# iqbal-lab-org/gramtools

Measured on AMD Instinct MI355X. Metric: 150bp reads quasimapped/sec (whole node); bit-exact coverage, higher is better.
Workload: dtype u32

## Files before the change

gramtools_amd/csrc/gmx_engine_cover_kernels.h:

```cpp
#pragma once
struct CoverAcc {
  uint32_t *acc;
  uint32_t *log;
  uint32_t *log_cursor;
  uint32_t log_cap;
  uint32_t *scratch_big;
  uint32_t n_lanes_big;
  int rng_mode;
  uint32_t log_sites;
  uint32_t *heap;
  uint64_t heap_words;
  const uint32_t *status;
  uint32_t n_tasks;
  unsigned long long *stats;
};

#define GMX_LOG_PAD 0xFFFFFFFFu
#ifdef GMX_LOOP_STATS
__device__ unsigned long long gmx_cover_stats[6 * 16];
__device__ unsigned long long gmx_coop_stats[6 * 8];
extern "C" int gmx_debug_coop_stats(unsigned long long *out, int reset) {
  if (hipMemcpyFromSymbol(out, HIP_SYMBOL(gmx_coop_stats), sizeof(gmx_coop_stats)) != hipSuccess) return -1;
  if (reset) {
    unsigned long long z[6 * 8] = {0};
// ... 800 lines not shown
    c[GMX_CNT_LOG_RETRY_HUGE * GMX_CNT_STRIDE] = 0;
  }
}
template <bool NESTED>
__global__ void __launch_bounds__(GMX_BLOCK) gmx_cover_single_replay_kernel(GmxIndexView ix, BatchView b, SearchOut o, CoverAcc acc,
                                                                            const uint32_t *recs_in) {
  const uint32_t n = o.counters[GMX_CNT_REPLAY_RECS * GMX_CNT_STRIDE];
  for (uint32_t i = blockIdx.x * GMX_BLOCK + threadIdx.x; i < n; i += gridDim.x * GMX_BLOCK)
    gmx_cover_single_rec<NESTED>(ix, o, acc, recs_in[i], o.cover_overflow_list, 4u);
}

__global__ void gmx_stats_limbs_kernel(unsigned long long *stats, uint32_t *limbs, int recombine) {
  const uint32_t t = threadIdx.x;
  if (!recombine) {
    if (t < 20) limbs[t] = (uint32_t)((stats[t >> 2] >> (16 * (t & 3))) & 0xFFFFull);
    else if (t < 32) limbs[t] = 0;
  } else if (t < 5) {
    unsigned long long v = 0;
    for (int l = 3; l >= 0; --l) v = (v << 16) + limbs[4 * t + l];
    stats[t] = v;
  }
}

#define GMX_PACK_READS 128
#define GMX_PACK_IN_BYTES (24 * 1024)
#define GMX_PACK_OUT_PAIRS (GMX_PACK_IN_BYTES / 32 + GMX_PACK_READS + 8)
typedef uint32_t __attribute__((aligned(1))) gmx_u32_unaligned;
__device__ __forceinline__ void pack4(uint32_t x, uint32_t &lo, uint32_t &hi, uint32_t &bad) {
  uint32_t y = x - 0x01010101u;
  bad |= ((y & ~x & 0x80808080u) | (y & 0xFCFCFCFCu));
  lo = (((y & 0x01010101u) * 0x01020408u) >> 24) & 0xFu;
  hi = ((((y >> 1) & 0x01010101u) * 0x01020408u) >> 24) & 0xFu;
}
__device__ __forceinline__ uint2 pack_tail(const uint8_t *p, uint32_t rem, uint32_t &bad) {
  uint2 out = make_uint2(0, 0);
  for (uint32_t j = 0; j < rem; ++j) {
    uint32_t x = p[j];
    if (x < 1 || x > 4) bad = 1;
    out.x |= ((x - 1u) & 1u) << j;
    out.y |= (((x - 1u) >> 1) & 1u) << j;
  }
  return out;
}
#define GMX_PACK_THREADS (2 * GMX_PACK_READS)
__global__ void __launch_bounds__(GMX_PACK_THREADS) gmx_pack_kernel(BatchView b, uint8_t *skip, uint2 *packed, uint32_t *counters,
                                                                    uint32_t *zero, uint32_t zero_words) {
// ... 86 lines not shown
```

gramtools_amd/csrc/gmx_engine_host.h:

```cpp
#pragma once
#define HIP_TRY(expr)                                                                      \
  do {                                                                                     \
    hipError_t _e = (expr);                                                                \
    if (_e != hipSuccess) {                                                                \
      gmx_set_error(std::string(#expr) + ": " + hipGetErrorString(_e));                    \
      return GMX_EHIP;                                                                     \
    }                                                                                      \
  } while (0)

enum : int { GMX_TK_SEED = 0, GMX_TK_FILTER0, GMX_TK_FILTER1, GMX_TK_SINGLE, GMX_TK_EXTEND2, GMX_TK_UNPACK, GMX_TK_N };
static_assert(GMX_TK_N <= GMX_TIMED_KERNELS, "gmx_timing::kernel_ms holds GMX_TIMED_KERNELS entries");

struct gmx_engine {
  gmx_engine_opts opts;
  GmxIndexView dview;
  std::vector<void *> allocs;
  uint64_t index_bytes = 0;
  uint32_t *d_fused = nullptr, *d_limbs = nullptr;
  size_t n_fused = 0, n_acc = 0;
  std::vector<uint32_t> phys_allele, phys_pb, phys_grouped;
  std::vector<uint32_t> hit_fix;
  unsigned long long *d_stats = nullptr;
  uint32_t *d_error = nullptr;
  uint32_t *d_log = nullptr, *d_log_cursor = nullptr;
  uint32_t log_cap = 0;
  uint32_t n_allele = 0, n_pb = 0, n_grouped = 0;
  uint64_t cap_reads = 0;
  uint8_t *d_skip = nullptr;
  uint2 *d_packed = nullptr;
  uint64_t cap_packed = 0;
  uint32_t *d_status = nullptr, *d_n_final = nullptr, *d_mapped = nullptr, *d_overflow = nullptr, *d_counters = nullptr;
  uint32_t *d_general_rest = nullptr;
  uint32_t *d_single_rest = nullptr;
  bool cover_jump = false;
  uint32_t *d_task_lists = nullptr;
  GmxSeed *d_alive_seed = nullptr;
  uint32_t *d_alive = nullptr, *d_dead = nullptr, *d_dead2 = nullptr;
  uint64_t *d_seed_cursor = nullptr;
  bool seed_cursor = false;
  GmxFinalState *d_finals = nullptr;
  GmxPathNode *d_arena = nullptr;
  GmxCoverRec *d_cover_recs = nullptr;
  BigOut big{};
  uint32_t *d_scratch_big = nullptr, *d_cover_overflow = nullptr;
  uint32_t cover_big_lanes = 0;
// ... 3 lines not shown
  uint32_t inst_cap = 0;
  GmxPathNode *d_inst_arena = nullptr;
  GmxFinalState *d_inst_states = nullptr;
  uint32_t *d_inst_first = nullptr, *d_inst_width = nullptr;
  uint32_t *d_inst_serial = nullptr, *d_general_serial = nullptr, *d_big_serial = nullptr, *d_overflow3 = nullptr;
  bool coop = true;
  uint32_t *d_heap = nullptr;
  uint64_t heap_words = 0;
  bool log_sites = false;
  std::map<std::vector<uint32_t>, uint64_t> log_counts;
  uint32_t *h_log_state = nullptr;
  hipEvent_t ev_log_state = nullptr;
  bool log_state_pending = false;
  uint32_t *d_log_retry[2] = {nullptr, nullptr}, *d_log_retry_recs[2] = {nullptr, nullptr}, *d_log_retry_huge[2] = {nullptr, nullptr};
  int log_retry_side = 0;
  BatchView last_b{};
  SearchOut last_o{};
  CoverAcc last_acc{};
  size_t last_big_lds = 0;
  uint64_t log_replays = 0, log_replayed_entries = 0;
  uint64_t log_known = 0;
  uint64_t log_reads_since = 0;
  bool reset_pending = false;
  hipStream_t reset_stream = nullptr;
  hipStream_t side2_stream = nullptr;
  hipEvent_t ev_fork2 = nullptr, ev_side1 = nullptr, ev_filter = nullptr;
  hipStream_t side_stream = nullptr;
  hipEvent_t ev_fork = nullptr, ev_join = nullptr;
  hipEvent_t ev_wait = nullptr;
  struct GmxDeviceIndex *shared_index = nullptr;
  uint32_t filter_lds_words = 0;
  const uint32_t *d_kmer_planar = nullptr;
  const uint32_t *d_absent = nullptr;
  uint32_t n_absent = 0;
  bool use_absent = false;
  uint32_t n_cus = 256;
  uint32_t probe_iters = GMX_PROBE_ITERS;
  uint32_t extend_cap = 0;
  uint32_t extend_budget = 8;
  bool seeds_in_place = false;
  gmx_engine *twin = nullptr;
  gmx_engine *owner = nullptr;
  bool is_twin = false, twin_off = false;
  bool record_outcomes = false;
  uint32_t *d_outcomes = nullptr;
  uint64_t outcome_cap = 0, outcome_count = 0;
// ... 16 lines not shown
  uint64_t *d_offsets = nullptr;
  uint32_t *d_seeds = nullptr;
  uint64_t cap_bases = 0, cap_stage_reads = 0;
  struct StageSlot {
    uint8_t *d_reads = nullptr;
    uint64_t *d_offsets = nullptr, *h_offsets = nullptr;
    uint32_t *d_seeds = nullptr, *h_seeds = nullptr;
    uint64_t cap_bases = 0, cap_reads = 0;
    hipEvent_t copied = nullptr, done = nullptr;
    bool busy = false;
  } stage[2];
  hipStream_t copy_stream = nullptr;
  hipStream_t copy_stream2 = nullptr;
  uint32_t copy_toggle = 0;
  hipStream_t last_stream = nullptr;
  struct PackSlot {
    uint2 *d_planes = nullptr;
    uint64_t *d_offsets = nullptr;
    uint32_t *d_seeds = nullptr;
    uint8_t *d_skip = nullptr;
    uint64_t cap_pairs = 0, cap_reads = 0;
    hipEvent_t copied = nullptr, done = nullptr;
    bool busy = false;
  } pslot[3];
  uint32_t pslot_next = 0;
  void release(void *q) {
    if (!q) return;
    for (size_t i = 0; i < allocs.size(); ++i)
      if (allocs[i] == q) {
        allocs[i] = allocs.back();
        allocs.pop_back();
        (void)hipFree(q);
        return;
      }
  }
  bool timing = false;
  struct EvTriple { hipEvent_t s, a, b, c; uint64_t reads; hipEvent_t k[GMX_TIMED_KERNELS][2]; uint32_t timed; };
  std::vector<EvTriple> pending;
  double search_ms = 0, cover_ms = 0;
  uint64_t search_launches = 0, cover_launches = 0, timed_reads = 0;
  double kernel_ms[GMX_TIMED_KERNELS] = {0};
  uint64_t kernel_launches[GMX_TIMED_KERNELS] = {0};

  template <class T>
  int alloc(T **p, size_t count, bool zero) {
    void *q = nullptr;
    size_t bytes = std::max<size_t>(count, 1) * sizeof(T);
    allocs.reserve(allocs.size() + 1);
// ... 56 lines not shown
  }
  return GMX_OK;
}

static int note_zeroed(gmx_engine *e, hipStream_t stream) {
  if (!e->twin) return GMX_OK;
  if (!e->ev_zeroed) HIP_TRY(hipEventCreateWithFlags(&e->ev_zeroed, hipEventDisableTiming));
  HIP_TRY(hipEventRecord(e->ev_zeroed, stream));
  ++e->zero_epoch;
  return GMX_OK;
}
static int twin_join(gmx_engine *e, hipStream_t stream) {
  gmx_engine *tw = e->twin;
  if (!tw || !e->twin_in_flight) return GMX_OK;
  if (!e->ev_twin_done) HIP_TRY(hipEventCreateWithFlags(&e->ev_twin_done, hipEventDisableTiming));
  HIP_TRY(hipEventRecord(e->ev_twin_done, tw->main_stream));
  HIP_TRY(hipStreamWaitEvent(stream, e->ev_twin_done, 0));
  return GMX_OK;
}
static int flush_reset(gmx_engine *e) {
  if (!e->reset_pending) return GMX_OK;
  e->reset_pending = false;
  HIP_TRY(hipMemsetAsync(e->d_fused, 0, (e->n_fused + 32) * 4, e->reset_stream));
  return note_zeroed(e, e->reset_stream);
}

static int log_settle(gmx_engine *e);
static int gmx_log_drain(gmx_engine *e, uint64_t keep_below) {
  int frc = flush_reset(e);
  if (frc) return frc;
  HIP_TRY(hipDeviceSynchronize());
  uint32_t used = 0;
  HIP_TRY(hipMemcpy(&used, e->d_log_cursor, 4, hipMemcpyDeviceToHost));
  used = std::min(used, e->log_cap);
  e->log_reads_since = 0;
  e->log_known = used;
  if (used <= keep_below) return GMX_OK;
  std::vector<uint32_t> w(used);
  HIP_TRY(hipMemcpy(w.data(), e->d_log, (size_t)used * 4, hipMemcpyDeviceToHost));
  std::vector<uint32_t> key;
  for (size_t i = 0; i < w.size();) {
    if (w[i] == GMX_LOG_PAD) {
      ++i;
      continue;
    }
    if (i + 2 > w.size() || i + 2 + (size_t)w[i + 1] > w.size()) {
      gmx_set_error("grouped-allele-count log: malformed record at word " + std::to_string(i) + " of " + std::to_string(w.size()));
      return GMX_EREF;
// ... 432 lines not shown
    return GMX_EHIP;
  }
  *out = e;
  return GMX_OK;
}

void gmx_engine_destroy(gmx_engine *e) try {
  if (!e) return;
  (void)hipSetDevice(e->opts.device);
  (void)hipDeviceSynchronize();
  if (e->twin) gmx_engine_destroy(e->twin);
  e->twin = nullptr;
  if (e->main_stream) (void)hipStreamDestroy(e->main_stream);
  if (e->ev_zeroed) (void)hipEventDestroy(e->ev_zeroed);
  if (e->ev_twin_done) (void)hipEventDestroy(e->ev_twin_done);
  if (e->side_stream) (void)hipStreamDestroy(e->side_stream);
  if (e->side2_stream) (void)hipStreamDestroy(e->side2_stream);
  if (e->ev_fork2) (void)hipEventDestroy(e->ev_fork2);
  if (e->ev_side1) (void)hipEventDestroy(e->ev_side1);
  if (e->ev_filter) (void)hipEventDestroy(e->ev_filter);
  if (e->ev_fork) (void)hipEventDestroy(e->ev_fork);
  if (e->ev_join) (void)hipEventDestroy(e->ev_join);
  if (e->ev_wait) (void)hipEventDestroy(e->ev_wait);
  if (e->copy_stream) (void)hipStreamDestroy(e->copy_stream);
  if (e->copy_stream2) (void)hipStreamDestroy(e->copy_stream2);
  if (e->h_log_state) (void)hipHostFree(e->h_log_state);
  if (e->ev_log_state) (void)hipEventDestroy(e->ev_log_state);
  for (auto &sl : e->pslot) {
    if (sl.copied) (void)hipEventDestroy(sl.copied);
    if (sl.done) (void)hipEventDestroy(sl.done);
  }
  for (auto &sl : e->stage) {
    if (sl.copied) (void)hipEventDestroy(sl.copied);
    if (sl.done) (void)hipEventDestroy(sl.done);
    if (sl.h_offsets) (void)hipHostFree(sl.h_offsets);
    if (sl.h_seeds) (void)hipHostFree(sl.h_seeds);
  }
  for (void *p : e->allocs) (void)hipFree(p);
  if (e->d_outcomes) (void)hipFree(e->d_outcomes);
  gmx_dev_index_release(e->shared_index);
  delete e;
} GMX_GUARD_VOID("gmx_engine_destroy")

int gmx_engine_reset(gmx_engine *e) try {
  HIP_TRY(hipSetDevice(e->opts.device));
  e->reset_pending = false;
  HIP_TRY(hipDeviceSynchronize());
  HIP_TRY(hipMemset(e->d_fused, 0, (e->n_fused + 32) * 4));
  HIP_TRY(hipMemset(e->d_error, 0, 8));
  HIP_TRY(hipMemset(e->d_counters, 0, GMX_N_COUNTERS * GMX_CNT_STRIDE * 4));
  if (e->twin) {
    HIP_TRY(hipMemset(e->twin->d_error, 0, 8));
    HIP_TRY(hipMemset(e->twin->d_counters, 0, GMX_N_COUNTERS * GMX_CNT_STRIDE * 4));
    e->twin_in_flight = false;
  }
  if (e->outcome_count) HIP_TRY(hipMemset(e->d_outcomes, 0, (e->outcome_count + 3) & ~3ull));
  e->outcome_count = 0;
  ++e->outcome_epoch;
  e->log_counts.clear();
  e->log_known = e->log_reads_since = 0;
  e->log_state_pending = false;
  return GMX_OK;
} GMX_GUARD_INT("gmx_engine_reset")

int gmx_engine_reset_async(gmx_engine *e, void *hip_stream) try {
  HIP_TRY(hipSetDevice(e->opts.device));
  hipStream_t st = (hipStream_t)hip_stream;
  int frc = flush_reset(e);
  if (frc) return frc;
  if ((frc = twin_join(e, st))) return frc;
  e->twin_in_flight = false;
  if (e->outcome_count) HIP_TRY(hipMemsetAsync(e->d_outcomes, 0, (e->outcome_count + 3) & ~3ull, st));
  e->outcome_count = 0;
  ++e->outcome_epoch;
  e->reset_pending = true;
  e->reset_stream = st;
  e->log_counts.clear();
  e->log_known = e->log_reads_since = 0;
  e->log_state_pending = false;
  return GMX_OK;
} GMX_GUARD_INT("gmx_engine_reset_async")

static bool gmx_ab_no_filter() {
  static const bool off = getenv("GMX_AB_NO_FILTER") != nullptr;
  return off;
}
static void launch_filter(gmx_engine *e, hipStream_t st, dim3 task_grid, const BatchView &b, const SearchOut &o, int pass,
                          hipEvent_t t0 = nullptr, hipEvent_t t1 = nullptr) {
  if (gmx_ab_no_filter()) return;
  if (e->filter_lds_words)
    hipExtLaunchKernelGGL(gmx_filter_lds_kernel, dim3(e->n_cus), dim3(GMX_FILTER_LDS_THREADS), e->filter_lds_words * 4,
                          st, t0, t1, 0u, e->dview, b, o, e->d_kmer_planar, e->filter_lds_words, pass);
  else if (e->use_absent)
    hipExtLaunchKernelGGL(gmx_filter_absent_kernel, task_grid, dim3(GMX_BLOCK), 0, st, t0, t1, 0u, e->dview, b, o, e->d_absent, e->n_absent, pass);
  else
    hipExtLaunchKernelGGL(gmx_filter_kernel, task_grid, dim3(GMX_BLOCK), 0, st, t0, t1, 0u, e->dview, b, o, pass);
}

static int log_state_enqueue(gmx_engine *e, hipStream_t stream) {
  if (!e->h_log_state) {
    HIP_TRY(hipHostMalloc(reinterpret_cast<void **>(&e->h_log_state), 4 * sizeof(uint32_t), hipHostMallocDefault));
    HIP_TRY(hipEventCreateWithFlags(&e->ev_log_state, hipEventDisableTiming));
  }
// ... 27 lines not shown
  e->last_o.log_retry_list = o.log_retry_list;
  e->last_o.log_retry_recs = o.log_retry_recs;
  e->last_o.log_retry_huge = o.log_retry_huge;
  return log_state_enqueue(e, stream);
}

static int log_settle(gmx_engine *e) {
  if (!e->log_state_pending) return GMX_OK;
  uint64_t before = ~0ull;
  for (int round = 0;; ++round) {
    HIP_TRY(hipEventSynchronize(e->ev_log_state));
    e->log_state_pending = false;
    const uint32_t used = std::min(e->h_log_state[0], e->log_cap);
    const uint64_t retries = (uint64_t)e->h_log_state[1] + e->h_log_state[2] + e->h_log_state[3];
    if (retries == 0) {
      if (used > e->log_cap / 2) return gmx_log_drain(e, 0);
      e->log_known = used;
      return GMX_OK;
    }
    if (round > 0 && retries >= before) {
      HIP_TRY(hipDeviceSynchronize());
      const uint32_t err[2] = {GMX_TASK_LOGFULL, 0};
      HIP_TRY(hipMemcpy(e->d_error, err, 8, hipMemcpyHostToDevice));
      return GMX_OK;
    }
    before = retries;
    int rc = gmx_log_drain(e, 0);
    if (rc) return rc;
    e->log_replays++;
    e->log_replayed_entries += retries;
    if ((rc = launch_log_replay(e, e->last_stream))) return rc;
  }
}

struct BatchInput {
  const uint8_t *d_reads = nullptr;
  const uint64_t *d_offsets = nullptr;
  const uint32_t *d_seeds = nullptr;
  const uint2 *d_planes = nullptr;
  const uint8_t *d_skip = nullptr;
  const uint32_t *d_twobit = nullptr;
  uint32_t twobit_base0 = 0;
  uint32_t uniform_len = 0;
  uint64_t n_reads = 0, total_bases = 0;
};

// ... 38 lines not shown
      const uint64_t w = j >> 4;
      const uint32_t sh = (uint32_t)(j & 15u) * 2u;
      const uint32_t w0 = stream[w], w1 = stream[w + 1], w2 = stream[w + 2];
      const unsigned long long bits = (unsigned long long)__builtin_amdgcn_alignbit(w1, w0, sh) |
                                      ((unsigned long long)__builtin_amdgcn_alignbit(w2, w1, sh) << 32);
      out[p] = make_uint2(gmx_even_bits(bits), gmx_even_bits(bits >> 1));
    }
  }
}

static int launch_batch(gmx_engine *e, const BatchInput &in, hipStream_t stream) {
  const uint64_t n_reads = in.n_reads, total_bases = in.total_bases;
  if (n_reads == 0) return GMX_OK;
  if (n_reads > (0x7fffffffull / GMX_FAST_ARENA) / 2) {
    gmx_set_error("batch too large: at most 44 M reads per launch (lower gmx_engine_opts.max_batch_reads)");
    return GMX_EINVAL;
  }
  int rc = e->log_sites ? log_settle(e) : GMX_OK;
  if (rc) return rc;
  if ((rc = ensure_batch_capacity(e, n_reads, true))) return rc;
  const bool fold_reset = e->reset_pending && e->reset_stream == stream;
  if (e->reset_pending && !fold_reset && (rc = flush_reset(e))) return rc;
  e->reset_pending = false;
  if (!in.d_planes) {
    uint64_t need = total_bases / 32 + n_reads + 16;
    if (need > e->cap_packed) {
      rc = e->alloc(&e->d_packed, need, false);
      if (rc) return rc;
      e->cap_packed = need;
    }
  }
  BatchView b{in.d_reads, in.d_offsets, in.d_seeds, (in.d_planes || in.d_twobit) ? in.d_skip : e->d_skip, in.d_planes ? in.d_planes : e->d_packed,
              (uint32_t)n_reads, (uint32_t)(e->opts.forward_only ? 1 : 0), in.uniform_len, (in.uniform_len + 31u) / 32u,
              e->keep_states ? 1u : 0u};
  const uint32_t region_inv = (uint32_t)std::min<uint64_t>(0xFFFFFFFFull, (((uint64_t)GMX_REGIONS << 32) + e->dview.n_prg - 1) / std::max<uint32_t>(e->dview.n_prg, 1u));
  SearchOut o{};
  o.status = e->d_status;
  o.n_final = e->d_n_final;
  o.finals = e->d_finals;
  o.arena = e->d_arena;
  o.cover_recs = e->d_cover_recs;
  o.cover_rec_task = e->d_mapped;
  o.region_cap = (uint32_t)(e->cap_reads * 2);
  o.region_inv = region_inv;
  o.task_lists = e->d_task_lists;
  o.list_stride = (uint32_t)(e->cap_reads * 2);
// ... 380 lines not shown
static int pick_target(gmx_engine *e, BatchTarget *out) {
  out->eng = e;
  out->stream = nullptr;
  e->last_on_twin = false;
  gmx_engine *tw = e->twin;
  if (!tw || e->twin_off || e->keep_states) return GMX_OK;
  if (e->reset_pending) {
    e->twin_toggle = 1;
    return GMX_OK;
  }
  if ((e->twin_toggle++ & 1u) == 0) return GMX_OK;
  if (tw->seen_zero_epoch != e->zero_epoch) {
    HIP_TRY(hipStreamWaitEvent(tw->main_stream, e->ev_zeroed, 0));
    tw->seen_zero_epoch = e->zero_epoch;
  }
  tw->timing = e->timing;
  out->eng = tw;
  out->stream = tw->main_stream;
  e->twin_in_flight = true;
  e->last_on_twin = true;
  return GMX_OK;
}

static int map_reads_packed_impl(gmx_engine *e, const uint64_t *planes, bool twobit, const uint64_t *offsets, uint32_t uniform_len,
                                 const uint32_t *seeds, const uint8_t *skip, uint64_t n_reads) {
  if (!e || !planes || !seeds || (!offsets && !uniform_len)) {
    gmx_set_error("gmx_map_reads_packed_host / gmx_map_reads_2bit_host: null argument (offsets may be null only with uniform_len)");
    return GMX_EINVAL;
  }
  if (n_reads == 0) return GMX_OK;
  HIP_TRY(hipSetDevice(e->opts.device));
  if (!e->copy_stream) HIP_TRY(hipStreamCreateWithFlags(&e->copy_stream, hipStreamNonBlocking));
  static const bool two_copy_streams = getenv("GMX_TWO_COPY_STREAMS") != nullptr;
  if (two_copy_streams && !e->copy_stream2) HIP_TRY(hipStreamCreateWithFlags(&e->copy_stream2, hipStreamNonBlocking));
  const uint32_t ppr = (uniform_len + 31u) / 32u;
  auto base_at = [&](uint64_t r) -> uint64_t { return uniform_len ? r * uniform_len : offsets[r] - offsets[0]; };
  auto pair_at = [&](uint64_t r) -> uint64_t {
    if (twobit) return (base_at(r) + 31) >> 5;
    return uniform_len ? r * ppr : ((offsets[r] >> 5) - (offsets[0] >> 5)) + r;
  };
  struct Reg { const void *p; bool on; };
  Reg regs[4] = {{planes, false}, {offsets, false}, {seeds, false}, {skip, false}};
  const uint64_t reg_bytes[4] = {pair_at(n_reads) * 8, (n_reads + 1) * 8, n_reads * 4, n_reads};
  bool all_pinned = true;
  for (int i = 0; i < 4; ++i) {
    if (!regs[i].p || gmx_is_pinned(regs[i].p)) continue;
    regs[i].on = hipHostRegister(const_cast<void *>(regs[i].p), reg_bytes[i], hipHostRegisterDefault) == hipSuccess;
    (void)hipGetLastError();
    all_pinned = false;
  }
  const uint32_t *d_seeds_host = nullptr;
  if (e->seeds_in_place && gmx_is_pinned(seeds)) {
    void *dp = nullptr;
    if (hipHostGetDevicePointer(&dp, const_cast<uint32_t *>(seeds), 0) == hipSuccess && dp) d_seeds_host = static_cast<const uint32_t *>(dp);
    else (void)hipGetLastError();
  }
  const uint64_t chunk = gmx_feed_chunk(e);
  int rc = GMX_OK;
  auto hip_ok = [&](hipError_t err, const char *what) {
    if (err == hipSuccess) return true;
    gmx_set_error(std::string(what) + ": " + hipGetErrorString(err));
    rc = GMX_EHIP;
    return false;
  };
  try {
  for (uint64_t done = 0; done < n_reads && rc == GMX_OK;) {
    gmx_engine::PackSlot &sl = e->pslot[e->pslot_next];
    e->pslot_next = (e->pslot_next + 1) % 3;
    const uint64_t n = std::min<uint64_t>(chunk, n_reads - done);
    uint64_t p0 = pair_at(done), pairs = pair_at(done + n) - p0;
    uint32_t twobit_base0 = 0;
    if (twobit) {
      const uint64_t b0 = base_at(done), b1 = base_at(done + n);
      p0 = b0 >> 5;
      pairs = ((b1 + 31) >> 5) - p0;
      twobit_base0 = (uint32_t)(b0 & 31u);
    }
    if (sl.busy) {
      if (!hip_ok(gmx_event_wait(sl.done), "hipEventSynchronize")) break;
      sl.busy = false;
    }
    if (!sl.copied) {
      if (!hip_ok(hipEventCreateWithFlags(&sl.copied, hipEventDisableTiming | hipEventBlockingSync), "hipEventCreate") ||
          !hip_ok(hipEventCreateWithFlags(&sl.done, hipEventDisableTiming | hipEventBlockingSync), "hipEventCreate"))
        break;
    }
    if (pairs + 16 > sl.cap_pairs) {
      const uint64_t cp = pairs + pairs / 8 + 64;
      e->release(sl.d_planes);
      sl.d_planes = nullptr;
      sl.cap_pairs = 0;
      if ((rc = e->alloc(&sl.d_planes, cp, false))) break;
      sl.cap_pairs = cp;
    }
    if (n > sl.cap_reads) {
      const uint64_t cr = std::max<uint64_t>(n, 1024);
      e->release(sl.d_offsets);
      e->release(sl.d_seeds);
      e->release(sl.d_skip);
      sl.d_offsets = nullptr;
      sl.d_seeds = nullptr;
      sl.d_skip = nullptr;
      sl.cap_reads = 0;
      if ((rc = e->alloc(&sl.d_offsets, cr + 1, false)) || (rc = e->alloc(&sl.d_seeds, cr, false)) || (rc = e->alloc(&sl.d_skip, cr, false))) break;
      sl.cap_reads = cr;
    }
    const hipStream_t cs = two_copy_streams && ((e->copy_toggle++) & 1u) ? e->copy_stream2 : e->copy_stream;
    if (!hip_ok(hipMemcpyAsync(sl.d_planes, planes + p0, pairs * 8, hipMemcpyHostToDevice, cs), "hipMemcpyAsync(planes)")) break;
    if (!uniform_len &&
        !hip_ok(hipMemcpyAsync(sl.d_offsets, offsets + done, (n + 1) * 8, hipMemcpyHostToDevice, cs), "hipMemcpyAsync(offsets)"))
      break;
    if (!d_seeds_host &&
        !hip_ok(hipMemcpyAsync(sl.d_seeds, seeds + done, n * 4, hipMemcpyHostToDevice, cs), "hipMemcpyAsync(seeds)"))
      break;
    if (skip && !hip_ok(hipMemcpyAsync(sl.d_skip, skip + done, n, hipMemcpyHostToDevice, cs), "hipMemcpyAsync(skip)")) break;
    BatchTarget tg;
    if ((rc = pick_target(e, &tg))) break;
    if (!hip_ok(hipEventRecord(sl.copied, cs), "hipEventRecord") ||
        !hip_ok(hipStreamWaitEvent(tg.stream, sl.copied, 0), "hipStreamWaitEvent"))
      break;
    BatchInput in;
    in.d_offsets = uniform_len ? nullptr : sl.d_offsets;
    in.d_seeds = d_seeds_host ? d_seeds_host + done : sl.d_seeds;
    in.d_planes = twobit ? nullptr : sl.d_planes;
    in.d_twobit = twobit ? reinterpret_cast<const uint32_t *>(sl.d_planes) : nullptr;
    in.twobit_base0 = twobit_base0;
    in.d_skip = skip ? sl.d_skip : nullptr;
    in.uniform_len = uniform_len;
    in.n_reads = n;
    in.total_bases = uniform_len ? n * (uint64_t)uniform_len : offsets[done + n] - offsets[done];
    if ((rc = launch_batch(tg.eng, in, tg.stream))) break;
    if (!hip_ok(hipEventRecord(sl.done, tg.stream), "hipEventRecord")) break;
    sl.busy = true;
    done += n;
  }
  } catch (...) {
    rc = gmx_guard_catch(twobit ? "gmx_map_reads_2bit_host" : "gmx_map_reads_packed_host");
  }
  if (rc != GMX_OK || !all_pinned) {
    (void)hipStreamSynchronize(e->copy_stream);
    if (e->copy_stream2) (void)hipStreamSynchronize(e->copy_stream2);
    if (rc != GMX_OK) {
      (void)hipDeviceSynchronize();
      for (auto &sl : e->pslot) sl.busy = false;
    }
  }
  for (int i = 0; i < 4; ++i)
    if (regs[i].on) (void)hipHostUnregister(const_cast<void *>(regs[i].p));
  (void)hipGetLastError();
  return rc;
}

int gmx_map_reads_packed_host(gmx_engine *e, const uint64_t *planes, const uint64_t *offsets, uint32_t uniform_len,
                              const uint32_t *seeds, const uint8_t *skip, uint64_t n_reads) try {
  return map_reads_packed_impl(e, planes, false, offsets, uniform_len, seeds, skip, n_reads);
} GMX_GUARD_INT("gmx_map_reads_packed_host")

// ... 153 lines not shown
  }
  if (n_bases > e->cap_bases) {
    if ((rc = e->alloc(&e->d_reads, n_bases + 16, false))) return rc;
    e->cap_bases = n_bases;
  }
  if (n_reads > e->cap_stage_reads) {
    if ((rc = e->alloc(&e->d_offsets, n_reads + 1, false)) || (rc = e->alloc(&e->d_seeds, n_reads, false))) return rc;
    e->cap_stage_reads = n_reads;
  }
  return GMX_OK;
} GMX_GUARD_INT("gmx_engine_reserve")

int gmx_engine_reserve_packed(gmx_engine *e, uint64_t n_reads, uint64_t n_pairs) try {
  if (!e) {
    gmx_set_error("null engine");
    return GMX_EINVAL;
  }
  HIP_TRY(hipSetDevice(e->opts.device));
  n_reads = std::min<uint64_t>(n_reads, gmx_feed_chunk(e));
  int rc = ensure_batch_capacity(e, n_reads);
  if (rc) return rc;
  if (e->twin && (rc = ensure_batch_capacity(e->twin, n_reads))) return rc;
  if (!e->copy_stream) HIP_TRY(hipStreamCreateWithFlags(&e->copy_stream, hipStreamNonBlocking));
  for (auto &sl : e->pslot) {
    if (sl.busy) continue;
    if (!sl.copied) {
      HIP_TRY(hipEventCreateWithFlags(&sl.copied, hipEventDisableTiming | hipEventBlockingSync));
      HIP_TRY(hipEventCreateWithFlags(&sl.done, hipEventDisableTiming | hipEventBlockingSync));
    }
    if (n_pairs + 16 > sl.cap_pairs) {
      e->release(sl.d_planes);
      sl.d_planes = nullptr;
      sl.cap_pairs = 0;
      if ((rc = e->alloc(&sl.d_planes, n_pairs + 64, false))) return rc;
      sl.cap_pairs = n_pairs + 64;
    }
    if (n_reads > sl.cap_reads) {
      e->release(sl.d_offsets);
      e->release(sl.d_seeds);
      e->release(sl.d_skip);
      sl.d_offsets = nullptr;
      sl.d_seeds = nullptr;
      sl.d_skip = nullptr;
      sl.cap_reads = 0;
      if ((rc = e->alloc(&sl.d_offsets, n_reads + 1, false)) || (rc = e->alloc(&sl.d_seeds, n_reads, false)) ||
          (rc = e->alloc(&sl.d_skip, n_reads, false)))
        return rc;
// ... 127 lines not shown
  out->cover_general = c(8);
  out->cover_mid = c(13);
  out->cover_overflow = c(4);
  out->seed_cursor = e->seed_cursor ? 1 : 0;
  out->inst_mapped = c(25);
  out->huge_search = c(11);
  out->huge_cover = c(15);
  out->log_replays = e->log_replays;
  out->log_replayed_entries = e->log_replayed_entries;
  out->overflow_split = c(29);
  return GMX_OK;
} GMX_GUARD_INT("gmx_engine_queue_counts")

int gmx_coverage_device(gmx_engine *e, gmx_device_coverage *out) try {
  {
    int frc = flush_reset(e);
    if (frc) return frc;
  }
  if (e->twin && e->twin_in_flight) {
    int qrc = gmx_quiesce(e->twin);
    if (qrc) return qrc;
    e->twin_in_flight = false;
  }
  out->allele_sum = out->per_base = out->grouped = nullptr;
  out->n_allele_sum = e->n_allele;
  out->n_per_base = e->n_pb;
  out->n_grouped = e->n_grouped;
  out->stats = e->d_stats;
  out->n_stats = 5;
  out->fused = e->d_fused;
  out->n_fused = e->n_fused;
  return GMX_OK;
} GMX_GUARD_INT("gmx_coverage_device")

int gmx_coverage_reduce_begin(gmx_engine *e, void *hip_stream) try {
  if (!e) {
    gmx_set_error("null engine");
    return GMX_EINVAL;
  }
  {
    int frc = flush_reset(e);
    if (frc) return frc;
    if ((frc = log_settle(e))) return frc;
  }
  HIP_TRY(hipSetDevice(e->opts.device));
  {
    int trc = twin_join(e, (hipStream_t)hip_stream);
    if (trc) return trc;
  }
  hipLaunchKernelGGL(gmx_stats_limbs_kernel, dim3(1), dim3(64), 0, (hipStream_t)hip_stream, e->d_stats, e->d_limbs, 0);
  HIP_TRY(hipGetLastError());
  return GMX_OK;
} GMX_GUARD_INT("gmx_coverage_reduce_begin")

int gmx_coverage_reduce_end(gmx_engine *e, void *hip_stream) try {
  if (!e) {
    gmx_set_error("null engine");
    return GMX_EINVAL;
  }
  {
    int frc = flush_reset(e);
    if (frc) return frc;
  }
  HIP_TRY(hipSetDevice(e->opts.device));
  hipLaunchKernelGGL(gmx_stats_limbs_kernel, dim3(1), dim3(64), 0, (hipStream_t)hip_stream, e->d_stats, e->d_limbs, 1);
  HIP_TRY(hipGetLastError());
  return GMX_OK;
} GMX_GUARD_INT("gmx_coverage_reduce_end")

int gmx_coverage_fetch(gmx_engine *e, uint32_t *allele_sum, uint32_t *per_base, uint32_t *grouped, gmx_stats *stats) try {
  if (!e) {
    gmx_set_error("null engine");
    return GMX_EINVAL;
  }
  {
    int frc = flush_reset(e);
    if (frc) return frc;
    if ((frc = log_settle(e))) return frc;
  }
  HIP_TRY(hipSetDevice(e->opts.device));
  HIP_TRY(hipDeviceSynchronize());
  std::vector<uint32_t> block(std::max<size_t>(e->n_acc, 1));
  if (e->n_acc) HIP_TRY(hipMemcpy(block.data(), e->d_fused, e->n_acc * 4, hipMemcpyDeviceToHost));
  if (allele_sum) for (size_t i = 0; i < e->phys_allele.size(); ++i) allele_sum[i] = block[e->phys_allele[i]];
  if (per_base) for (size_t i = 0; i < e->phys_pb.size(); ++i) per_base[i] = block[e->phys_pb[i]];
  if (grouped) for (size_t i = 0; i < e->phys_grouped.size(); ++i) grouped[i] = block[e->phys_grouped[i]];
  for (size_t i = 0; i + 3 < e->hit_fix.size(); i += 4) {
    const uint32_t hits = block[e->hit_fix[i]];
    if (allele_sum) allele_sum[e->hit_fix[i + 1]] += hits;
    if (grouped) grouped[e->hit_fix[i + 2]] += hits;
    if (per_base) per_base[e->hit_fix[i + 3]] += hits;
  }
  if (stats) {
    unsigned long long s[5];
    HIP_TRY(hipMemcpy(s, e->d_stats, sizeof(s), hipMemcpyDeviceToHost));
    stats->all_reads_count = s[0];
    stats->skipped_reads_count = s[1];
    stats->missing_kmer_reads_count = s[2];
    stats->no_extension_reads_count = s[3];
    stats->exact_mapped_reads_count = s[4];
  }
  return GMX_OK;
} GMX_GUARD_INT("gmx_coverage_fetch")

int gmx_engine_record_outcomes(gmx_engine *e, int on) try {
  if (!e) {
    gmx_set_error("null engine");
    return GMX_EINVAL;
  }
  e->record_outcomes = on != 0;
  return GMX_OK;
} GMX_GUARD_INT("gmx_engine_record_outcomes")

int64_t gmx_engine_outcome_count(gmx_engine *e) try {
  if (!e) {
    gmx_set_error("null engine");
    return GMX_EINVAL;
  }
  return (int64_t)e->outcome_count;
} GMX_GUARD_INT("gmx_engine_outcome_count")

int gmx_engine_fetch_outcomes(gmx_engine *e, uint64_t first, uint64_t n, uint8_t *out) try {
  if (!e || (n && !out)) {
    gmx_set_error("gmx_engine_fetch_outcomes: null argument");
    return GMX_EINVAL;
  }
  if (first > e->outcome_count || n > e->outcome_count - first) {
    gmx_set_error("gmx_engine_fetch_outcomes: reads " + std::to_string(first) + " .. " + std::to_string(first + n) + " of " +
                  std::to_string(e->outcome_count) + " recorded");
    return GMX_EINVAL;
  }
  {
    int frc = flush_reset(e);
    if (frc) return frc;
    if ((frc = log_settle(e))) return frc;
  }
  HIP_TRY(hipSetDevice(e->opts.device));
  HIP_TRY(hipDeviceSynchronize());
  if (n) HIP_TRY(hipMemcpy(out, reinterpret_cast<const uint8_t *>(e->d_outcomes) + first, n, hipMemcpyDeviceToHost));
  return GMX_OK;
} GMX_GUARD_INT("gmx_engine_fetch_outcomes")

int64_t gmx_coverage_fetch_grouped_log(gmx_engine *e, uint32_t *out, uint64_t cap_words) try {
  if (!e) return GMX_EINVAL;
  if (hipSetDevice(e->opts.device) != hipSuccess) return GMX_EHIP;
  if (log_settle(e)) return GMX_EHIP;
  if (gmx_log_drain(e, 0)) return GMX_EHIP;
  uint64_t n = 0;
  for (auto const &kv : e->log_counts) {
    const uint64_t words = 4 + (kv.first.size() - 1);
    if (out && n + words <= cap_words) {
      out[n] = kv.first[0];
      out[n + 1] = (uint32_t)(kv.first.size() - 1) | GMX_LOG_COUNTED;
      out[n + 2] = (uint32_t)kv.second;
      out[n + 3] = (uint32_t)(kv.second >> 32);
      for (size_t j = 1; j < kv.first.size(); ++j) out[n + 3 + j] = kv.first[j];
    }
    n += words;
  }
  return (int64_t)n;
} GMX_GUARD_INT("gmx_coverage_fetch_grouped_log")

int gmx_coverage_import_grouped_log(gmx_engine *e, const uint32_t *records, uint64_t n_words, int replace) try {
  if (!e || (!records && n_words)) {
    gmx_set_error("gmx_coverage_import_grouped_log: null argument");
    return GMX_EINVAL;
  }
  {
    int frc = flush_reset(e);
    if (frc) return frc;
  }
  HIP_TRY(hipSetDevice(e->opts.device));
  return gmx_engine_log_import(e, records, (size_t)n_words, replace != 0);
} GMX_GUARD_INT("gmx_coverage_import_grouped_log")

}

uint64_t gmx_engine_outcome_epoch(const gmx_engine *e) { return e->outcome_epoch; }

void gmx_engine_raw(gmx_engine *e, GmxEngineRaw *out) {
  (void)flush_reset(e);
  out->device = e->opts.device;
  out->d_fused = e->d_fused;
  out->n_fused = e->n_fused;
  out->log_sites = e->log_sites;
}

int gmx_engine_log_export(gmx_engine *e, std::vector<uint32_t> &out) {
  {
    int frc = flush_reset(e);
    if (frc) return frc;
    if ((frc = log_settle(e))) return frc;
  }
  const int64_t n = gmx_coverage_fetch_grouped_log(e, nullptr, 0);
  if (n < 0) return (int)n;
  out.assign((size_t)n, 0);
  if (n && gmx_coverage_fetch_grouped_log(e, out.data(), (uint64_t)n) < 0) return GMX_EHIP;
  return GMX_OK;
}

int gmx_engine_log_import(gmx_engine *e, const uint32_t *w, size_t n_words, bool replace) {
  {
    int frc = flush_reset(e);
    if (frc) return frc;
// ... 30 lines not shown
```

include/gmx.h:

```cpp
#ifndef GMX_H
#define GMX_H
#include <stddef.h>
#include <stdint.h>

#ifdef __cplusplus
extern "C" {
#endif

#define GMX_OK 0
#define GMX_EINVAL (-1)
#define GMX_ENODEV (-2)
#define GMX_EHIP (-3)
#define GMX_ECAP (-4)
#define GMX_EREF (-5)
#define GMX_ENOMEM (-6)

typedef struct gmx_index gmx_index;
typedef struct gmx_engine gmx_engine;

const char *gmx_last_error(void);

int gmx_index_build(const uint32_t *prg, uint64_t n_symbols, uint32_t kmer_size, int threads, gmx_index **out);
int gmx_index_build_from_file(const char *prg_path, uint32_t kmer_size, int threads, gmx_index **out);
int gmx_index_save(const gmx_index *ix, const char *path);
// ... 43 lines not shown
int64_t gmx_index_jump_states(const gmx_index *ix, uint32_t lo, uint32_t hi, int64_t *out, uint64_t cap);

typedef struct gmx_engine_opts {
  int device;
  int rng_mode;
  uint32_t max_states;
  uint32_t max_path_nodes;
  uint64_t max_batch_reads;
  int forward_only;
  uint64_t huge_heap_bytes;
  uint64_t log_cap_words;
} gmx_engine_opts;
void gmx_engine_default_opts(gmx_engine_opts *opts);

int gmx_engine_create(const gmx_index *ix, const gmx_engine_opts *opts, gmx_engine **out);
void gmx_engine_destroy(gmx_engine *e);
int gmx_engine_reset(gmx_engine *e);
int gmx_engine_reset_async(gmx_engine *e, void *hip_stream);

int gmx_map_reads_host(gmx_engine *e, const uint8_t *reads, const uint64_t *offsets, const uint32_t *seeds,
                       uint64_t n_reads);
int gmx_map_reads_device(gmx_engine *e, const uint8_t *d_reads, const uint64_t *d_offsets, const uint32_t *d_seeds,
                         uint64_t n_reads, uint64_t total_bases, void *hip_stream);
int gmx_map_reads_packed_host(gmx_engine *e, const uint64_t *planes, const uint64_t *offsets, uint32_t uniform_len,
                              const uint32_t *seeds, const uint8_t *skip, uint64_t n_reads);
int gmx_engine_sync_uploads(gmx_engine *e);
int gmx_engine_seeds_in_place(gmx_engine *e, int on);
uint64_t gmx_packed_pairs(const uint64_t *offsets, uint32_t uniform_len, uint64_t n_reads);
int gmx_pack_reads(const uint8_t *reads, const uint64_t *offsets, uint32_t uniform_len, uint64_t n_reads, uint64_t *planes,
                   uint8_t *skip, int threads);
int gmx_map_reads_2bit_host(gmx_engine *e, const uint64_t *stream, const uint64_t *offsets, uint32_t uniform_len,
                            const uint32_t *seeds, const uint8_t *skip, uint64_t n_reads);
uint64_t gmx_twobit_units(const uint64_t *offsets, uint32_t uniform_len, uint64_t n_reads);
int gmx_pack_reads_2bit(const uint8_t *reads, const uint64_t *offsets, uint32_t uniform_len, uint64_t n_reads, uint64_t *stream,
                        uint8_t *skip, int threads);
int gmx_map_reads_packed_device(gmx_engine *e, const uint64_t *d_planes, const uint64_t *d_offsets, uint32_t uniform_len,
                                const uint32_t *seeds, const uint8_t *d_skip, uint64_t n_reads);
void *gmx_engine_second_stream(gmx_engine *e);

typedef struct gmx_ingest gmx_ingest;
typedef struct {
  uint64_t offset;
  uint32_t size;
  uint32_t isize;
  uint32_t crc32;
  uint32_t reserved;
// ... 203 lines not shown
```

Measured before the change: 1.457 billion.

## Gather coverage on device, make reset async, deepen pack ring, add host tracing

Moves the coverage fetch gather from the host to a GPU kernel that writes a compact pinned output with the stats appended. The old path copied the whole accumulator block back and gathered on the CPU. Reset now queues async memsets instead of blocking memsets and defers the host wait to the next flush. The packed-read upload ring grows from 3 to 4 slots (settable by env), and the grouped-log drain is skipped when there is no log state. It also adds env-gated host timing traces, at the cost of more state flags and a one-time setup of device-side index tables.

```diff
diff --git a/gramtools_amd/csrc/gmx_engine_cover_kernels.h b/gramtools_amd/csrc/gmx_engine_cover_kernels.h
--- a/gramtools_amd/csrc/gmx_engine_cover_kernels.h
+++ b/gramtools_amd/csrc/gmx_engine_cover_kernels.h
@@ -846,6 +846,18 @@
   }
 }
 
+__global__ void __launch_bounds__(256) gmx_fetch_gather_kernel(const uint32_t *__restrict__ block, const uint32_t *__restrict__ src,
+                                                               const uint32_t *__restrict__ fix_start, const uint32_t *__restrict__ fix_src,
+                                                               uint32_t n_out, const unsigned long long *__restrict__ stats,
+                                                               uint32_t *__restrict__ out) {
+  for (uint32_t i = blockIdx.x * blockDim.x + threadIdx.x; i < n_out; i += gridDim.x * blockDim.x) {
+    uint32_t v = block[src[i]];
+    for (uint32_t j = fix_start[i], j1 = fix_start[i + 1]; j < j1; ++j) v += block[fix_src[j]];
+    out[i] = v;
+  }
+  if (blockIdx.x == 0 && threadIdx.x < 10) out[n_out + threadIdx.x] = (uint32_t)(stats[threadIdx.x >> 1] >> (32 * (threadIdx.x & 1)));
+}
+
 #define GMX_PACK_READS 128
 #define GMX_PACK_IN_BYTES (24 * 1024)
 #define GMX_PACK_OUT_PAIRS (GMX_PACK_IN_BYTES / 32 + GMX_PACK_READS + 8)
diff --git a/gramtools_amd/csrc/gmx_engine_host.h b/gramtools_amd/csrc/gmx_engine_host.h
--- a/gramtools_amd/csrc/gmx_engine_host.h
+++ b/gramtools_amd/csrc/gmx_engine_host.h
@@ -21,6 +21,11 @@
   std::vector<uint32_t> phys_allele, phys_pb, phys_grouped;
   std::vector<uint32_t> hit_fix;
   unsigned long long *d_stats = nullptr;
+  uint32_t *d_fetch_src = nullptr, *d_fetch_fix_start = nullptr, *d_fetch_fix_src = nullptr, *d_fetch_out = nullptr;
+  uint32_t *h_fetch = nullptr;
+  hipEvent_t ev_fetch = nullptr;
+  bool fetch_ready = false;
+  bool foreign_streams = false;
   uint32_t *d_error = nullptr;
   uint32_t *d_log = nullptr, *d_log_cursor = nullptr;
   uint32_t log_cap = 0;
@@ -70,6 +75,7 @@
   uint64_t log_known = 0;
   uint64_t log_reads_since = 0;
   bool reset_pending = false;
+  bool reset_host_wait = false;
   hipStream_t reset_stream = nullptr;
   hipStream_t side2_stream = nullptr;
   hipEvent_t ev_fork2 = nullptr, ev_side1 = nullptr, ev_filter = nullptr;
@@ -132,8 +138,9 @@
     uint64_t cap_pairs = 0, cap_reads = 0;
     hipEvent_t copied = nullptr, done = nullptr;
     bool busy = false;
-  } pslot[3];
+  } pslot[GMX_PACK_SLOTS_MAX];
   uint32_t pslot_next = 0;
+  uint32_t n_pslots = GMX_PACK_SLOTS;
   void release(void *q) {
     if (!q) return;
     for (size_t i = 0; i < allocs.size(); ++i)
@@ -236,8 +243,28 @@
   if (!e->reset_pending) return GMX_OK;
   e->reset_pending = false;
   HIP_TRY(hipMemsetAsync(e->d_fused, 0, (e->n_fused + 32) * 4, e->reset_stream));
-  return note_zeroed(e, e->reset_stream);
-}
+  const int rc = note_zeroed(e, e->reset_stream);
+  if (e->reset_host_wait) HIP_TRY(hipStreamSynchronize(e->reset_stream));
+  e->reset_host_wait = false;
+  return rc;
+}
+
+static bool gmx_host_trace_on() {
+  static const bool on = getenv("GMX_FEED_TRACE") != nullptr;
+  return on;
+}
+static double gmx_host_trace_us() {
+  static const auto t0 = std::chrono::steady_clock::now();
+  return std::chrono::duration<double, std::micro>(std::chrono::steady_clock::now() - t0).count();
+}
+#define GMX_HOST_TRACE(...)                                     \
+  do {                                                          \
+    if (gmx_host_trace_on()) {                                  \
+      fprintf(stderr, "[gmx %12.1f] ", gmx_host_trace_us());    \
+      fprintf(stderr, __VA_ARGS__);                             \
+      fputc('\n', stderr);                                      \
+    }                                                           \
+  } while (0)
 
 static int log_settle(gmx_engine *e);
 static int gmx_log_drain(gmx_engine *e, uint64_t keep_below) {
@@ -716,6 +743,8 @@
   if (e->ev_fork) (void)hipEventDestroy(e->ev_fork);
   if (e->ev_join) (void)hipEventDestroy(e->ev_join);
   if (e->ev_wait) (void)hipEventDestroy(e->ev_wait);
+  if (e->ev_fetch) (void)hipEventDestroy(e->ev_fetch);
+  if (e->h_fetch) (void)hipHostFree(e->h_fetch);
   if (e->copy_stream) (void)hipStreamDestroy(e->copy_stream);
   if (e->copy_stream2) (void)hipStreamDestroy(e->copy_stream2);
   if (e->h_log_state) (void)hipHostFree(e->h_log_state);
@@ -736,33 +765,9 @@
   delete e;
 } GMX_GUARD_VOID("gmx_engine_destroy")
 
-int gmx_engine_reset(gmx_engine *e) try {
-  HIP_TRY(hipSetDevice(e->opts.device));
-  e->reset_pending = false;
-  HIP_TRY(hipDeviceSynchronize());
-  HIP_TRY(hipMemset(e->d_fused, 0, (e->n_fused + 32) * 4));
-  HIP_TRY(hipMemset(e->d_error, 0, 8));
-  HIP_TRY(hipMemset(e->d_counters, 0, GMX_N_COUNTERS * GMX_CNT_STRIDE * 4));
-  if (e->twin) {
-    HIP_TRY(hipMemset(e->twin->d_error, 0, 8));
-    HIP_TRY(hipMemset(e->twin->d_counters, 0, GMX_N_COUNTERS * GMX_CNT_STRIDE * 4));
-    e->twin_in_flight = false;
-  }
-  if (e->outcome_count) HIP_TRY(hipMemset(e->d_outcomes, 0, (e->outcome_count + 3) & ~3ull));
-  e->outcome_count = 0;
-  ++e->outcome_epoch;
-  e->log_counts.clear();
-  e->log_known = e->log_reads_since = 0;
-  e->log_state_pending = false;
-  return GMX_OK;
-} GMX_GUARD_INT("gmx_engine_reset")
-
-int gmx_engine_reset_async(gmx_engine *e, void *hip_stream) try {
-  HIP_TRY(hipSetDevice(e->opts.device));
-  hipStream_t st = (hipStream_t)hip_stream;
-  int frc = flush_reset(e);
-  if (frc) return frc;
-  if ((frc = twin_join(e, st))) return frc;
+static int queue_reset(gmx_engine *e, hipStream_t st) {
+  int rc = twin_join(e, st);
+  if (rc) return rc;
   e->twin_in_flight = false;
   if (e->outcome_count) HIP_TRY(hipMemsetAsync(e->d_outcomes, 0, (e->outcome_count + 3) & ~3ull, st));
   e->outcome_count = 0;
@@ -773,6 +778,36 @@
   e->log_known = e->log_reads_since = 0;
   e->log_state_pending = false;
   return GMX_OK;
+}
+
+int gmx_engine_reset(gmx_engine *e) try {
+  HIP_TRY(hipSetDevice(e->opts.device));
+  const double t0 = gmx_host_trace_on() ? gmx_host_trace_us() : 0;
+  e->reset_pending = false;
+  HIP_TRY(hipDeviceSynchronize());
+  const double t1 = gmx_host_trace_on() ? gmx_host_trace_us() : 0;
+  e->twin_in_flight = false;
+  HIP_TRY(hipMemsetAsync(e->d_error, 0, 8, nullptr));
+  HIP_TRY(hipMemsetAsync(e->d_counters, 0, GMX_N_COUNTERS * GMX_CNT_STRIDE * 4, nullptr));
+  if (e->twin) {
+    HIP_TRY(hipMemsetAsync(e->twin->d_error, 0, 8, nullptr));
+    HIP_TRY(hipMemsetAsync(e->twin->d_counters, 0, GMX_N_COUNTERS * GMX_CNT_STRIDE * 4, nullptr));
+  }
+  const int rc = queue_reset(e, nullptr);
+  e->reset_host_wait = true;
+  GMX_HOST_TRACE("reset: wait %.1f us, queue %.1f us", t1 - t0, gmx_host_trace_us() - t1);
+  return rc;
+} GMX_GUARD_INT("gmx_engine_reset")
+
+int gmx_engine_reset_async(gmx_engine *e, void *hip_stream) try {
+  HIP_TRY(hipSetDevice(e->opts.device));
+  hipStream_t st = (hipStream_t)hip_stream;
+  if (st) e->foreign_streams = true;
+  int frc = flush_reset(e);
+  if (frc) return frc;
+  frc = queue_reset(e, st);
+  e->reset_host_wait = false;
+  return frc;
 } GMX_GUARD_INT("gmx_engine_reset_async")
 
 static bool gmx_ab_no_filter() {
@@ -846,6 +881,7 @@
       HIP_TRY(hipDeviceSynchronize());
       const uint32_t err[2] = {GMX_TASK_LOGFULL, 0};
       HIP_TRY(hipMemcpy(e->d_error, err, 8, hipMemcpyHostToDevice));
+      e->log_known = used;
       return GMX_OK;
     }
     before = retries;
@@ -930,6 +966,8 @@
   const bool fold_reset = e->reset_pending && e->reset_stream == stream;
   if (e->reset_pending && !fold_reset && (rc = flush_reset(e))) return rc;
   e->reset_pending = false;
+  e->reset_host_wait = false;
+  if (stream && !e->is_twin) e->foreign_streams = true;
   if (!in.d_planes) {
     uint64_t need = total_bases / 32 + n_reads + 16;
     if (need > e->cap_packed) {
@@ -1356,6 +1394,19 @@
   return GMX_OK;
 }
 
+static void gmx_pack_ring_depth(gmx_engine *e) {
+  static const uint32_t depth = [] {
+    const char *env = getenv("GMX_FEED_SLOTS");
+    const long v = env ? atol(env) : (long)GMX_PACK_SLOTS;
+    return (uint32_t)std::min<long>(std::max<long>(v, 2), GMX_PACK_SLOTS_MAX);
+  }();
+  if (depth == e->n_pslots) return;
+  for (auto &sl : e->pslot)
+    if (sl.busy) return;
+  e->n_pslots = depth;
+  e->pslot_next = 0;
+}
+
 static int map_reads_packed_impl(gmx_engine *e, const uint64_t *planes, bool twobit, const uint64_t *offsets, uint32_t uniform_len,
                                  const uint32_t *seeds, const uint8_t *skip, uint64_t n_reads) {
   if (!e || !planes || !seeds || (!offsets && !uniform_len)) {
@@ -1367,6 +1418,7 @@
   if (!e->copy_stream) HIP_TRY(hipStreamCreateWithFlags(&e->copy_stream, hipStreamNonBlocking));
   static const bool two_copy_streams = getenv("GMX_TWO_COPY_STREAMS") != nullptr;
   if (two_copy_streams && !e->copy_stream2) HIP_TRY(hipStreamCreateWithFlags(&e->copy_stream2, hipStreamNonBlocking));
+  gmx_pack_ring_depth(e);
   const uint32_t ppr = (uniform_len + 31u) / 32u;
   auto base_at = [&](uint64_t r) -> uint64_t { return uniform_len ? r * uniform_len : offsets[r] - offsets[0]; };
   auto pair_at = [&](uint64_t r) -> uint64_t {
@@ -1400,7 +1452,7 @@
   try {
   for (uint64_t done = 0; done < n_reads && rc == GMX_OK;) {
     gmx_engine::PackSlot &sl = e->pslot[e->pslot_next];
-    e->pslot_next = (e->pslot_next + 1) % 3;
+    e->pslot_next = (e->pslot_next + 1) % e->n_pslots;
     const uint64_t n = std::min<uint64_t>(chunk, n_reads - done);
     uint64_t p0 = pair_at(done), pairs = pair_at(done + n) - p0;
     uint32_t twobit_base0 = 0;
@@ -1411,8 +1463,10 @@
       twobit_base0 = (uint32_t)(b0 & 31u);
     }
     if (sl.busy) {
+      const double w0 = gmx_host_trace_on() ? gmx_host_trace_us() : 0;
       if (!hip_ok(gmx_event_wait(sl.done), "hipEventSynchronize")) break;
       sl.busy = false;
+      GMX_HOST_TRACE("feed: slot %u waited %.1f us", (unsigned)(&sl - e->pslot), gmx_host_trace_us() - w0);
     }
     if (!sl.copied) {
       if (!hip_ok(hipEventCreateWithFlags(&sl.copied, hipEventDisableTiming | hipEventBlockingSync), "hipEventCreate") ||
@@ -1440,7 +1494,9 @@
       sl.cap_reads = cr;
     }
     const hipStream_t cs = two_copy_streams && ((e->copy_toggle++) & 1u) ? e->copy_stream2 : e->copy_stream;
+    const double c0 = gmx_host_trace_on() ? gmx_host_trace_us() : 0;
     if (!hip_ok(hipMemcpyAsync(sl.d_planes, planes + p0, pairs * 8, hipMemcpyHostToDevice, cs), "hipMemcpyAsync(planes)")) break;
+    GMX_HOST_TRACE("feed: slot %u copy of %llu bytes queued in %.1f us", (unsigned)(&sl - e->pslot), (unsigned long long)(pairs * 8), gmx_host_trace_us() - c0);
     if (!uniform_len &&
         !hip_ok(hipMemcpyAsync(sl.d_offsets, offsets + done, (n + 1) * 8, hipMemcpyHostToDevice, cs), "hipMemcpyAsync(offsets)"))
       break;
@@ -1463,10 +1519,12 @@
     in.uniform_len = uniform_len;
     in.n_reads = n;
     in.total_bases = uniform_len ? n * (uint64_t)uniform_len : offsets[done + n] - offsets[done];
+    const double l0 = gmx_host_trace_on() ? gmx_host_trace_us() : 0;
     if ((rc = launch_batch(tg.eng, in, tg.stream))) break;
     if (!hip_ok(hipEventRecord(sl.done, tg.stream), "hipEventRecord")) break;
     sl.busy = true;
     done += n;
+    GMX_HOST_TRACE("feed: %llu reads launched in %.1f us", (unsigned long long)n, gmx_host_trace_us() - l0);
   }
   } catch (...) {
     rc = gmx_guard_catch(twobit ? "gmx_map_reads_2bit_host" : "gmx_map_reads_packed_host");
@@ -1666,7 +1724,9 @@
   if (rc) return rc;
   if (e->twin && (rc = ensure_batch_capacity(e->twin, n_reads))) return rc;
   if (!e->copy_stream) HIP_TRY(hipStreamCreateWithFlags(&e->copy_stream, hipStreamNonBlocking));
-  for (auto &sl : e->pslot) {
+  gmx_pack_ring_depth(e);
+  for (uint32_t si = 0; si < e->n_pslots; ++si) {
+    gmx_engine::PackSlot &sl = e->pslot[si];
     if (sl.busy) continue;
     if (!sl.copied) {
       HIP_TRY(hipEventCreateWithFlags(&sl.copied, hipEventDisableTiming | hipEventBlockingSync));
@@ -1840,6 +1900,7 @@
     if (qrc) return qrc;
     e->twin_in_flight = false;
   }
+  e->foreign_streams = true;
   out->allele_sum = out->per_base = out->grouped = nullptr;
   out->n_allele_sum = e->n_allele;
   out->n_per_base = e->n_pb;
@@ -1866,6 +1927,7 @@
     int trc = twin_join(e, (hipStream_t)hip_stream);
     if (trc) return trc;
   }
+  e->foreign_streams = true;
   hipLaunchKernelGGL(gmx_stats_limbs_kernel, dim3(1), dim3(64), 0, (hipStream_t)hip_stream, e->d_stats, e->d_limbs, 0);
   HIP_TRY(hipGetLastError());
   return GMX_OK;
@@ -1881,22 +1943,13 @@
     if (frc) return frc;
   }
   HIP_TRY(hipSetDevice(e->opts.device));
+  e->foreign_streams = true;
   hipLaunchKernelGGL(gmx_stats_limbs_kernel, dim3(1), dim3(64), 0, (hipStream_t)hip_stream, e->d_stats, e->d_limbs, 1);
   HIP_TRY(hipGetLastError());
   return GMX_OK;
 } GMX_GUARD_INT("gmx_coverage_reduce_end")
 
-int gmx_coverage_fetch(gmx_engine *e, uint32_t *allele_sum, uint32_t *per_base, uint32_t *grouped, gmx_stats *stats) try {
-  if (!e) {
-    gmx_set_error("null engine");
-    return GMX_EINVAL;
-  }
-  {
-    int frc = flush_reset(e);
-    if (frc) return frc;
-    if ((frc = log_settle(e))) return frc;
-  }
-  HIP_TRY(hipSetDevice(e->opts.device));
+static int coverage_fetch_host_gather(gmx_engine *e, uint32_t *allele_sum, uint32_t *per_base, uint32_t *grouped, gmx_stats *stats) {
   HIP_TRY(hipDeviceSynchronize());
   std::vector<uint32_t> block(std::max<size_t>(e->n_acc, 1));
   if (e->n_acc) HIP_TRY(hipMemcpy(block.data(), e->d_fused, e->n_acc * 4, hipMemcpyDeviceToHost));
@@ -1919,6 +1972,110 @@
     stats->exact_mapped_reads_count = s[4];
   }
   return GMX_OK;
+}
+
+static int coverage_fetch_prepare(gmx_engine *e) {
+  const size_t na = e->phys_allele.size(), np = e->phys_pb.size(), ng = e->phys_grouped.size(), n_out = na + np + ng;
+  const size_t words = std::max<size_t>(e->n_acc, 64);
+  std::vector<uint32_t> src;
+  src.reserve(n_out + 1);
+  src.insert(src.end(), e->phys_allele.begin(), e->phys_allele.end());
+  src.insert(src.end(), e->phys_pb.begin(), e->phys_pb.end());
+  src.insert(src.end(), e->phys_grouped.begin(), e->phys_grouped.end());
+  bool ok = n_out < 0xFFFFFFF0ull;
+  for (uint32_t w : src) ok = ok && w < words;
+  std::vector<uint32_t> start(n_out + 2, 0), fsrc;
+  const size_t base[3] = {0, na + np, na};
+  const size_t size[3] = {na, ng, np};
+  for (size_t i = 0; ok && i + 3 < e->hit_fix.size(); i += 4) {
+    ok = e->hit_fix[i] < words;
+    for (int k = 0; ok && k < 3; ++k) {
+      ok = e->hit_fix[i + 1 + k] < size[k];
+      if (ok) ++start[base[k] + e->hit_fix[i + 1 + k] + 1];
+    }
+  }
+  if (!ok) {
+    gmx_set_error("gmx_coverage_fetch: the index's coverage slot tables point outside its accumulator block");
+    return GMX_EREF;
+  }
+  for (size_t i = 0; i < n_out; ++i) start[i + 1] += start[i];
+  fsrc.assign(std::max<size_t>(start[n_out], 1), 0);
+  {
+    std::vector<uint32_t> at(start.begin(), start.begin() + n_out);
+    for (size_t i = 0; i + 3 < e->hit_fix.size(); i += 4)
+      for (int k = 0; k < 3; ++k) fsrc[at[base[k] + e->hit_fix[i + 1 + k]]++] = e->hit_fix[i];
+  }
+  if (src.empty()) src.push_back(0);
+  int rc;
+  if ((rc = e->alloc(&e->d_fetch_src, src.size(), false)) || (rc = e->alloc(&e->d_fetch_fix_start, start.size(), false)) ||
+      (rc = e->alloc(&e->d_fetch_fix_src, fsrc.size(), false)) || (rc = e->alloc(&e->d_fetch_out, n_out + 16, false)))
+    return rc;
+  HIP_TRY(hipMemcpy(e->d_fetch_src, src.data(), src.size() * 4, hipMemcpyHostToDevice));
+  HIP_TRY(hipMemcpy(e->d_fetch_fix_start, start.data(), start.size() * 4, hipMemcpyHostToDevice));
+  HIP_TRY(hipMemcpy(e->d_fetch_fix_src, fsrc.data(), fsrc.size() * 4, hipMemcpyHostToDevice));
+  HIP_TRY(hipHostMalloc(reinterpret_cast<void **>(&e->h_fetch), (n_out + 16) * 4, hipHostMallocDefault));
+  HIP_TRY(hipEventCreateWithFlags(&e->ev_fetch, hipEventDisableTiming | hipEventBlockingSync));
+  e->fetch_ready = true;
+  return GMX_OK;
+}
+
+int gmx_coverage_fetch(gmx_engine *e, uint32_t *allele_sum, uint32_t *per_base, uint32_t *grouped, gmx_stats *stats) try {
+  if (!e) {
+    gmx_set_error("null engine");
+    return GMX_EINVAL;
+  }
+  const bool trace = gmx_host_trace_on();
+  const double t0 = trace ? gmx_host_trace_us() : 0;
+  HIP_TRY(hipSetDevice(e->opts.device));
+  {
+    int frc = flush_reset(e);
+    if (frc) return frc;
+    if ((frc = log_settle(e))) return frc;
+  }
+  if (getenv("GMX_FETCH_HOST_GATHER")) {
+    const int rc = coverage_fetch_host_gather(e, allele_sum, per_base, grouped, stats);
+    GMX_HOST_TRACE("fetch (host gather): %.1f us", gmx_host_trace_us() - t0);
+    return rc;
+  }
+  if (!e->fetch_ready) {
+    const int prc = coverage_fetch_prepare(e);
+    if (prc) return prc;
+  }
+  const double t1 = trace ? gmx_host_trace_us() : 0;
+  hipStream_t st = e->last_stream;
+  if (e->foreign_streams) {
+    HIP_TRY(hipDeviceSynchronize());
+    st = nullptr;
+  } else {
+    const int trc = twin_join(e, st);
+    if (trc) return trc;
+  }
+  const double t2 = trace ? gmx_host_trace_us() : 0;
+  const size_t na = e->phys_allele.size(), np = e->phys_pb.size(), ng = e->phys_grouped.size(), n_out = na + np + ng;
+  const unsigned blocks = (unsigned)std::min<size_t>(std::max<size_t>((n_out + 255) / 256, 1), 4096);
+  hipLaunchKernelGGL(gmx_fetch_gather_kernel, dim3(blocks), dim3(256), 0, st, e->d_fused, e->d_fetch_src, e->d_fetch_fix_start,
+                     e->d_fetch_fix_src, (uint32_t)n_out, e->d_stats, e->d_fetch_out);
+  HIP_TRY(hipGetLastError());
+  HIP_TRY(hipMemcpyAsync(e->h_fetch, e->d_fetch_out, (n_out + 10) * 4, hipMemcpyDeviceToHost, st));
+  HIP_TRY(hipEventRecord(e->ev_fetch, st));
+  const double t3 = trace ? gmx_host_trace_us() : 0;
+  HIP_TRY(hipEventSynchronize(e->ev_fetch));
+  const double t4 = trace ? gmx_host_trace_us() : 0;
+  if (allele_sum && na) memcpy(allele_sum, e->h_fetch, na * 4);
+  if (per_base && np) memcpy(per_base, e->h_fetch + na, np * 4);
+  if (grouped && ng) memcpy(grouped, e->h_fetch + na + np, ng * 4);
+  if (stats) {
+    unsigned long long s[5];
+    memcpy(s, e->h_fetch + n_out, sizeof(s));
+    stats->all_reads_count = s[0];
+    stats->skipped_reads_count = s[1];
+    stats->missing_kmer_reads_count = s[2];
+    stats->no_extension_reads_count = s[3];
+    stats->exact_mapped_reads_count = s[4];
+  }
+  GMX_HOST_TRACE("fetch: settle %.1f us, order %.1f us, queue %.1f us, wait (kernels, gather, D2H of %zu bytes) %.1f us, copy out %.1f us",
+                 t1 - t0, t2 - t1, t3 - t2, (n_out + 10) * 4, t4 - t3, gmx_host_trace_us() - t4);
+  return GMX_OK;
 } GMX_GUARD_INT("gmx_coverage_fetch")
 
 int gmx_engine_record_outcomes(gmx_engine *e, int on) try {
@@ -1962,8 +2119,10 @@
 int64_t gmx_coverage_fetch_grouped_log(gmx_engine *e, uint32_t *out, uint64_t cap_words) try {
   if (!e) return GMX_EINVAL;
   if (hipSetDevice(e->opts.device) != hipSuccess) return GMX_EHIP;
+  const double t0 = gmx_host_trace_on() ? gmx_host_trace_us() : 0;
   if (log_settle(e)) return GMX_EHIP;
-  if (gmx_log_drain(e, 0)) return GMX_EHIP;
+  if (e->log_sites && (e->log_state_pending || e->log_known != 0) && gmx_log_drain(e, 0)) return GMX_EHIP;
+  GMX_HOST_TRACE("grouped log: settle + drain %.1f us", gmx_host_trace_us() - t0);
   uint64_t n = 0;
   for (auto const &kv : e->log_counts) {
     const uint64_t words = 4 + (kv.first.size() - 1);
@@ -1998,6 +2157,7 @@
 
 void gmx_engine_raw(gmx_engine *e, GmxEngineRaw *out) {
   (void)flush_reset(e);
+  e->foreign_streams = true;
   out->device = e->opts.device;
   out->d_fused = e->d_fused;
   out->n_fused = e->n_fused;
diff --git a/include/gmx.h b/include/gmx.h
--- a/include/gmx.h
+++ b/include/gmx.h
@@ -89,6 +89,8 @@
                        uint64_t n_reads);
 int gmx_map_reads_device(gmx_engine *e, const uint8_t *d_reads, const uint64_t *d_offsets, const uint32_t *d_seeds,
                          uint64_t n_reads, uint64_t total_bases, void *hip_stream);
+#define GMX_PACK_SLOTS 4
+#define GMX_PACK_SLOTS_MAX 6
 int gmx_map_reads_packed_host(gmx_engine *e, const uint64_t *planes, const uint64_t *offsets, uint32_t uniform_len,
                               const uint32_t *seeds, const uint8_t *skip, uint64_t n_reads);
 int gmx_engine_sync_uploads(gmx_engine *e);
```

Result: no change. 1.456 billion (-0.1%).
